# JasonLSC/GSCodec_Studio

Measured on AMD Instinct MI355X. Metric: Msplats/s fwd+bwd @1080p (1M splats), higher is better.
Workload: dtype f32; 1 GPU; BASELINE config 2: load_test_data(scene_grid=3) -> 1006065 gaussians, SH degree 3, 1x1 camera 1920x1080, packed=False, tile 16, fwd + bwd of sum(render); visible=292931, native_step_driver=True, parallelism=camera-sharded dp1

## Files before the change

gscodec_studio_amd/csrc/gs_common.h:

```cpp
#pragma once

#include <hip/hip_runtime.h>
#include <stdint.h>

#include "../../include/gsplat_hip.h"

#define GS_WAVE 64
#define GS_BLOCK 256

#define GS_DEV __device__ __forceinline__
#define GS_FP_STRICT _Pragma("clang fp contract(off)")

void gs_set_error(const char *fmt, ...);

#define GS_CHECK_ARG(cond, msg)                                                        \
    do {                                                                               \
        if (!(cond)) {                                                                 \
            gs_set_error("%s: %s", __func__, msg);                                     \
            return 1;                                                                  \
        }                                                                              \
    } while (0)

#define GS_CHECK_LAUNCH()                                                              \
    do {                                                                               \
        hipError_t e_ = hipGetLastError();                                             \
        if (e_ != hipSuccess) {                                                        \
            gs_set_error("%s: launch failed: %s", __func__, hipGetErrorString(e_));    \
            return 2;                                                                  \
        }                                                                              \
    } while (0)

static inline uint32_t gs_div_up(uint64_t a, uint64_t b) { return (uint32_t)((a + b - 1) / b); }

#define GS_PRESORT_BUCKETS 256
#ifdef __HIPCC__
__device__ __forceinline__ uint32_t gs_bucket_of(const uint64_t *s_split, uint64_t key) {
    uint32_t lo = 0;
#pragma unroll
    for (uint32_t step = GS_PRESORT_BUCKETS / 2; step >= 1; step >>= 1)
        if (s_split[lo + step - 1] <= key) lo += step;
    return lo;
}
#endif

#ifdef __HIPCC__
__device__ __forceinline__ float gs_mask_sigmoid(float v) { return __fdiv_rn(1.f, __fadd_rn(1.f, expf(-v))); }
__device__ __forceinline__ float gs_mask_value(float logit, float temperature, int binary) {
    if (binary) return gs_mask_sigmoid(logit) >= 0.5f ? 1.f : 0.f;
    return gs_mask_sigmoid(__fdiv_rn(logit, temperature));
}
#endif

#ifdef __HIPCC__
struct TileBox {
    int32_t x0, y0, x1, y1;
};
__device__ __forceinline__ TileBox tile_box(float mx, float my, int32_t radius, float tile_size, int32_t tw, int32_t th) {
    _Pragma("clang fp contract(off)");
    const float tr = ((float)radius / tile_size);
    const float tx = (mx / tile_size);
    const float ty = (my / tile_size);
    TileBox b;
    b.x0 = min(max(0, (int32_t)floorf((tx - tr))), tw);
    b.y0 = min(max(0, (int32_t)floorf((ty - tr))), th);
    b.x1 = min(max(0, (int32_t)ceilf((tx + tr))), tw);
    b.y1 = min(max(0, (int32_t)ceilf((ty + tr))), th);
    return b;
}
#endif

uint32_t *sort_first_hist_slot(uint64_t n, void *temp, size_t temp_bytes, uint32_t *n_blocks);

struct Vec3 {
    float x, y, z;
};
struct Mat3 {
    float m[3][3];
};
struct Sym3 {
    float xx, xy, xz, yy, yz, zz;
};
struct Sym2 {
    float xx, xy, yy;
};

GS_DEV Mat3 mat3_zero() {
    Mat3 r;
#pragma unroll
    for (int i = 0; i < 3; ++i)
#pragma unroll
        for (int j = 0; j < 3; ++j) r.m[i][j] = 0.f;
    return r;
}

GS_DEV Mat3 sym3_to_mat3(const Sym3 &s) {
    Mat3 r;
    r.m[0][0] = s.xx; r.m[0][1] = s.xy; r.m[0][2] = s.xz;
    r.m[1][0] = s.xy; r.m[1][1] = s.yy; r.m[1][2] = s.yz;
    r.m[2][0] = s.xz; r.m[2][1] = s.yz; r.m[2][2] = s.zz;
    return r;
}

GS_DEV Mat3 mat3_mul(const Mat3 &a, const Mat3 &b) {
    Mat3 r;
#pragma unroll
    for (int i = 0; i < 3; ++i)
#pragma unroll
        for (int j = 0; j < 3; ++j)
            r.m[i][j] = a.m[i][0] * b.m[0][j] + a.m[i][1] * b.m[1][j] + a.m[i][2] * b.m[2][j];
    return r;
}

GS_DEV Mat3 mat3_tmul(const Mat3 &a, const Mat3 &b) {
    Mat3 r;
#pragma unroll
    for (int i = 0; i < 3; ++i)
#pragma unroll
        for (int j = 0; j < 3; ++j)
            r.m[i][j] = a.m[0][i] * b.m[0][j] + a.m[1][i] * b.m[1][j] + a.m[2][i] * b.m[2][j];
    return r;
}

GS_DEV Mat3 mat3_mult(const Mat3 &a, const Mat3 &b) {
    Mat3 r;
#pragma unroll
    for (int i = 0; i < 3; ++i)
#pragma unroll
        for (int j = 0; j < 3; ++j)
            r.m[i][j] = a.m[i][0] * b.m[j][0] + a.m[i][1] * b.m[j][1] + a.m[i][2] * b.m[j][2];
    return r;
}

GS_DEV Sym3 sym3_congruence(const Mat3 &W, const Sym3 &S) {
    Mat3 Sm = sym3_to_mat3(S);
    Mat3 WS = mat3_mul(W, Sm);
    Sym3 r;
    r.xx = WS.m[0][0] * W.m[0][0] + WS.m[0][1] * W.m[0][1] + WS.m[0][2] * W.m[0][2];
    r.xy = WS.m[0][0] * W.m[1][0] + WS.m[0][1] * W.m[1][1] + WS.m[0][2] * W.m[1][2];
    r.xz = WS.m[0][0] * W.m[2][0] + WS.m[0][1] * W.m[2][1] + WS.m[0][2] * W.m[2][2];
    r.yy = WS.m[1][0] * W.m[1][0] + WS.m[1][1] * W.m[1][1] + WS.m[1][2] * W.m[1][2];
    r.yz = WS.m[1][0] * W.m[2][0] + WS.m[1][1] * W.m[2][1] + WS.m[1][2] * W.m[2][2];
    r.zz = WS.m[2][0] * W.m[2][0] + WS.m[2][1] * W.m[2][1] + WS.m[2][2] * W.m[2][2];
    return r;
}

GS_DEV Sym3 sym3_congruence_t(const Mat3 &W, const Sym3 &G) {
    Mat3 Gm = sym3_to_mat3(G);
    Mat3 GW = mat3_mul(Gm, W);
    Sym3 r;
    r.xx = W.m[0][0] * GW.m[0][0] + W.m[1][0] * GW.m[1][0] + W.m[2][0] * GW.m[2][0];
    r.xy = W.m[0][0] * GW.m[0][1] + W.m[1][0] * GW.m[1][1] + W.m[2][0] * GW.m[2][1];
    r.xz = W.m[0][0] * GW.m[0][2] + W.m[1][0] * GW.m[1][2] + W.m[2][0] * GW.m[2][2];
    r.yy = W.m[0][1] * GW.m[0][1] + W.m[1][1] * GW.m[1][1] + W.m[2][1] * GW.m[2][1];
    r.yz = W.m[0][1] * GW.m[0][2] + W.m[1][1] * GW.m[1][2] + W.m[2][1] * GW.m[2][2];
// ... 94 lines not shown
```

gscodec_studio_amd/csrc/isect.hip:

```cpp
#include "gs_common.h"

namespace {

__global__ void __launch_bounds__(GS_BLOCK) isect_count_kernel(
    uint32_t n_elems, const float *__restrict__ means2d, uint32_t s_m2, const int32_t *__restrict__ radii,
    float tile_size, int32_t tw, int32_t th, int32_t *__restrict__ tiles_per_gauss) {
    uint32_t i = blockIdx.x * GS_BLOCK + threadIdx.x;
    if (i >= n_elems) return;
    int32_t r = radii[i];
    int32_t cnt = 0;
    if (r > 0) {
        float2 m = *reinterpret_cast<const float2 *>(means2d + (size_t)i * s_m2);
        TileBox b = tile_box(m.x, m.y, r, tile_size, tw, th);
        cnt = (b.y1 - b.y0) * (b.x1 - b.x0);
    }
    tiles_per_gauss[i] = cnt;
}

__global__ void __launch_bounds__(GS_BLOCK) isect_depth_keys_kernel(
    uint32_t n_elems, const int32_t *__restrict__ radii, const float *__restrict__ depths,
    int64_t *__restrict__ keys, int32_t *__restrict__ vals) {
    uint32_t i = blockIdx.x * GS_BLOCK + threadIdx.x;
    if (i >= n_elems) return;
    uint32_t d = radii[i] > 0 ? (uint32_t)__float_as_int(depths[i]) & 0x7fffffffu : 0x7fffffffu;
    keys[i] = (int64_t)(((uint64_t)d << 32) | (uint64_t)i);
    vals[i] = (int32_t)i;
}

constexpr int COUNT_ITEMS = 4;
__global__ void __launch_bounds__(GS_BLOCK) isect_count_keys_kernel(
    uint32_t n_elems, const float *__restrict__ means2d, uint32_t s_m2, const int32_t *__restrict__ radii,
    const float *__restrict__ depths, float tile_size, int32_t tw, int32_t th,
    int32_t *__restrict__ tiles_per_gauss, int64_t *__restrict__ keys, int32_t *__restrict__ vals, int32_t *__restrict__ block_sums,
    uint32_t *__restrict__ hist, uint32_t n_blocks, const uint64_t *__restrict__ split) {
    __shared__ int32_t s_sum[GS_BLOCK / GS_WAVE], s_vis[GS_BLOCK / GS_WAVE];
    __shared__ uint32_t s_hist[256];
    __shared__ uint64_t s_split[GS_PRESORT_BUCKETS];
    if (hist != nullptr) s_hist[threadIdx.x] = 0u;
    if (split != nullptr) s_split[threadIdx.x] = split[threadIdx.x];
    __syncthreads();
    int32_t cnt_sum = 0, vis_sum = 0;
#pragma unroll
    for (int k = 0; k < COUNT_ITEMS; ++k) {
        const uint32_t i = (blockIdx.x * COUNT_ITEMS + k) * GS_BLOCK + threadIdx.x;
        if (i >= n_elems) continue;
        const int32_t r = radii[i];
        uint32_t d = 0x7fffffffu;
        int32_t cnt = 0;
        if (r > 0) {
            if (means2d != nullptr) {
                float2 m = *reinterpret_cast<const float2 *>(means2d + (size_t)i * s_m2);
                TileBox b = tile_box(m.x, m.y, r, tile_size, tw, th);
                cnt = (b.y1 - b.y0) * (b.x1 - b.x0);
            }
            d = (uint32_t)__float_as_int(depths[i]) & 0x7fffffffu;
        }
        if (means2d != nullptr) tiles_per_gauss[i] = cnt;
        const uint64_t key = ((uint64_t)d << 32) | (uint64_t)i;
        keys[i] = (int64_t)key;
        if (vals != nullptr) vals[i] = (int32_t)i;
        cnt_sum += cnt;
        vis_sum += r > 0 ? 1 : 0;
        if (hist != nullptr && d != 0x7fffffffu) atomicAdd(&s_hist[split != nullptr ? gs_bucket_of(s_split, key) : (d & 0xffu)], 1u);
    }
    if (block_sums != nullptr) {
        int32_t v = cnt_sum, u = vis_sum;
#pragma unroll
        for (int off = 32; off > 0; off >>= 1) {
            v += __shfl_xor(v, off, 64);
            u += __shfl_xor(u, off, 64);
        }
        if ((threadIdx.x & 63u) == 0u) {
            s_sum[threadIdx.x >> 6] = v;
            s_vis[threadIdx.x >> 6] = u;
        }
        __syncthreads();
        if (threadIdx.x == 0)
            reinterpret_cast<int2 *>(block_sums)[blockIdx.x] = make_int2(s_sum[0] + s_sum[1] + s_sum[2] + s_sum[3], s_vis[0] + s_vis[1] + s_vis[2] + s_vis[3]);
    }
    if (hist != nullptr) {
        __syncthreads();
        hist[(size_t)threadIdx.x * n_blocks + blockIdx.x] = s_hist[threadIdx.x];
    }
// ... 460 lines not shown
    hipLaunchKernelGGL(isect_emit_kernel<true>, dim3(gs_div_up(n_elems, EMIT_WAVES * EMIT_SPW)), dim3(GS_BLOCK), 0,
                       (hipStream_t)stream, n_elems, N, perm, n_valid, camera_ids, means2d, means2d_stride, radii, depths,
                       cum_tiles_per_gauss, (float)tile_size, (int32_t)tile_width, (int32_t)tile_height,
                       tile_n_bits, (int64_t *)nullptr, keys32, flatten_ids);
    GS_CHECK_LAUNCH();
    return 0;
}

extern "C" uint32_t gs_isect_emit_group_shift(void) { return EMIT_SCAN_SHIFT; }
extern "C" uint32_t gs_isect_emit_prefix_from_groups(void) { return 8192u; }

static int32_t emit_presorted_launch(
    int mode, uint32_t pos_bits, uint32_t n_elems, uint32_t N, const int32_t *perm, const uint32_t *n_valid, const int64_t *camera_ids,
    const float *means2d, uint32_t means2d_stride, const int32_t *radii, const float *depths, const int32_t *tiles_per_gauss,
    const uint32_t *group_sums, const int64_t *group_prefix, uint32_t tile_size, uint32_t tile_width, uint32_t tile_height,
    uint32_t tile_n_bits, int64_t *isect_ids, uint32_t *keys32, int32_t *flatten_ids, gs_stream_t stream) {
    const int32_t compact = mode != 0;
    if (n_elems == 0) return 0;
    GS_CHECK_ARG(means2d && radii && depths && tiles_per_gauss && (group_sums || group_prefix) && (flatten_ids || mode == 2), "null pointer");
    GS_CHECK_ARG(compact ? keys32 != nullptr : isect_ids != nullptr, "null output");
    GS_CHECK_ARG(camera_ids != nullptr || N > 0, "N must be > 0 when camera_ids is NULL");
    GS_CHECK_ARG(tile_n_bits < 32, "tile_n_bits must be < 32");
    GS_CHECK_ARG(means2d_stride >= 2 && means2d_stride % 2 == 0, "means2d_stride must be even and >= 2");
    GS_CHECK_ARG(n_elems < (1u << 31), "n_elems must be < 2^31");
    const dim3 grid(gs_div_up(n_elems, EMIT_SCAN_TILE));
    if (mode == 2)
        hipLaunchKernelGGL(isect_emit_scan_kernel<2>, grid, dim3(GS_BLOCK), 0, (hipStream_t)stream, n_elems, N, perm, n_valid, camera_ids,
                           means2d, means2d_stride, radii, depths, tiles_per_gauss, group_sums, group_prefix, (float)tile_size, (int32_t)tile_width,
                           (int32_t)tile_height, tile_n_bits, (int64_t *)nullptr, keys32, (int32_t *)nullptr, pos_bits);
    else if (compact)
        hipLaunchKernelGGL(isect_emit_scan_kernel<1>, grid, dim3(GS_BLOCK), 0, (hipStream_t)stream, n_elems, N, perm, n_valid, camera_ids,
                           means2d, means2d_stride, radii, depths, tiles_per_gauss, group_sums, group_prefix, (float)tile_size, (int32_t)tile_width,
                           (int32_t)tile_height, tile_n_bits, (int64_t *)nullptr, keys32, flatten_ids, 0u);
    else
        hipLaunchKernelGGL(isect_emit_scan_kernel<0>, grid, dim3(GS_BLOCK), 0, (hipStream_t)stream, n_elems, N, perm, n_valid, camera_ids,
                           means2d, means2d_stride, radii, depths, tiles_per_gauss, group_sums, group_prefix, (float)tile_size, (int32_t)tile_width,
                           (int32_t)tile_height, tile_n_bits, isect_ids, (uint32_t *)nullptr, flatten_ids, 0u);
    GS_CHECK_LAUNCH();
    return 0;
}

extern "C" int32_t gs_isect_emit_presorted(
    uint32_t n_elems, uint32_t N, const int32_t *perm, const uint32_t *n_valid, const int64_t *camera_ids, const float *means2d,
    uint32_t means2d_stride, const int32_t *radii, const float *depths, const int32_t *tiles_per_gauss, const uint32_t *group_sums,
    const int64_t *group_prefix, uint32_t tile_size, uint32_t tile_width, uint32_t tile_height, uint32_t tile_n_bits, int32_t compact,
    int64_t *isect_ids, uint32_t *keys32, int32_t *flatten_ids, gs_stream_t stream) {
    return emit_presorted_launch(compact ? 1 : 0, 0u, n_elems, N, perm, n_valid, camera_ids, means2d, means2d_stride, radii, depths,
                                 tiles_per_gauss, group_sums, group_prefix, tile_size, tile_width, tile_height, tile_n_bits, isect_ids, keys32,
                                 flatten_ids, stream);
}

extern "C" int32_t gs_isect_emit_packed(
    uint32_t n_elems, uint32_t N, const int32_t *perm, const uint32_t *n_valid, const int64_t *camera_ids, const float *means2d,
    uint32_t means2d_stride, const int32_t *radii, const float *depths, const int32_t *tiles_per_gauss, const uint32_t *group_sums,
    const int64_t *group_prefix, uint32_t tile_size, uint32_t tile_width, uint32_t tile_height, uint32_t tile_n_bits, uint32_t pos_bits,
    uint32_t *words, gs_stream_t stream) {
    GS_CHECK_ARG(pos_bits + tile_n_bits <= 32, "tile bits + position bits must fit 32 bits");
    return emit_presorted_launch(2, pos_bits, n_elems, N, perm, n_valid, camera_ids, means2d, means2d_stride, radii, depths, tiles_per_gauss,
                                 group_sums, group_prefix, tile_size, tile_width, tile_height, tile_n_bits, nullptr, words, nullptr, stream);
}

extern "C" int32_t gs_isect_offset_encode(
    uint32_t n_isects, const int64_t *isect_ids_sorted, uint32_t C, uint32_t n_tiles,
    uint32_t tile_n_bits, int32_t *offsets, gs_stream_t stream) {
    GS_CHECK_ARG(offsets != nullptr, "null pointer");
    if ((uint64_t)C * n_tiles == 0) return 0;
    if (n_isects == 0) {
        hipError_t e = hipMemsetAsync(offsets, 0, (size_t)C * n_tiles * sizeof(int32_t), (hipStream_t)stream);
        if (e != hipSuccess) {
            gs_set_error("gs_isect_offset_encode: memset failed: %s", hipGetErrorString(e));
            return 2;
        }
        return 0;
    }
    GS_CHECK_ARG(isect_ids_sorted != nullptr, "null pointer");
    hipLaunchKernelGGL(isect_offset_encode_kernel, dim3(gs_div_up(n_isects, GS_BLOCK * OFFSET_ITEMS)), dim3(GS_BLOCK), 0,
                       (hipStream_t)stream, n_isects, isect_ids_sorted, C, n_tiles, tile_n_bits, offsets);
    GS_CHECK_LAUNCH();
    return 0;
}

static size_t finish_pairs_bytes(uint64_t n) { return ((size_t)n * 4 + 255) / 256 * 256; }

extern "C" size_t gs_isect_finish_work_bytes(uint64_t n_isects) {
    return 2 * finish_pairs_bytes(n_isects) + gs_sort_isect_temp_bytes(n_isects);
}

extern "C" int32_t gs_isect_finish_presorted(
    uint32_t n_elems, uint32_t N, uint64_t n_isects, const int32_t *perm, const uint32_t *n_valid, const int64_t *camera_ids,
    const float *means2d, uint32_t means2d_stride, const int32_t *radii, const float *depths, const int32_t *tiles_per_gauss,
    const uint32_t *group_sums, const int64_t *group_prefix, uint32_t tile_size, uint32_t tile_width, uint32_t tile_height,
    uint32_t tile_n_bits, uint32_t cam_n_bits, uint32_t C, int64_t *isect_ids, int32_t *flatten_ids, int32_t *offsets, void *work,
    size_t work_bytes, uint32_t n_kept_host, const int64_t *sorted_keys, gs_stream_t stream) {
    GS_CHECK_ARG(offsets != nullptr, "null pointer");
    if (n_isects > 0) {
        GS_CHECK_ARG(work != nullptr && (uintptr_t)work % 16 == 0 && work_bytes >= gs_isect_finish_work_bytes(n_isects),
                     "work buffer too small (gs_isect_finish_work_bytes) or misaligned");
        const size_t pb = finish_pairs_bytes(n_isects);
        uint32_t *keys32 = (uint32_t *)work;
        int32_t *vals = (int32_t *)((char *)work + pb);
        void *temp = (char *)work + 2 * pb;
        uint32_t pos_bits = 0, cam_bits = 0;
        while (n_kept_host > 0 && ((uint64_t)1 << pos_bits) < (uint64_t)n_kept_host) ++pos_bits;
        while (((uint32_t)1 << cam_bits) < C) ++cam_bits;
        const uint32_t key_bits_eff = tile_n_bits + cam_bits;
        if (n_kept_host > 0 && perm != nullptr && camera_ids == nullptr && key_bits_eff >= 1 && key_bits_eff + pos_bits <= 32 &&
            key_bits_eff <= 31) {
            int32_t rc = gs_isect_emit_packed(n_elems, N, perm, n_valid, camera_ids, means2d, means2d_stride, radii, depths, tiles_per_gauss,
                                              group_sums, group_prefix, tile_size, tile_width, tile_height, tile_n_bits, pos_bits, keys32, stream);
            if (rc != 0) return rc;
            rc = gs_sort_isect_packed(n_isects, keys32, perm, sorted_keys, depths, (int32_t)key_bits_eff, pos_bits, isect_ids, flatten_ids,
                                      temp, work_bytes - 2 * pb, stream);
            if (rc != 0) return rc;
            return gs_isect_offset_encode((uint32_t)n_isects, isect_ids, C, tile_width * tile_height, tile_n_bits, offsets, stream);
        }
        int32_t rc = gs_isect_emit_presorted(n_elems, N, perm, n_valid, camera_ids, means2d, means2d_stride, radii, depths, tiles_per_gauss,
                                             group_sums, group_prefix, tile_size, tile_width, tile_height, tile_n_bits, 1, nullptr,
                                             keys32, vals, stream);
        if (rc != 0) return rc;
        const uint32_t sort_bits = (tile_n_bits + cam_n_bits < 32u && key_bits_eff >= 1u) ? key_bits_eff : tile_n_bits + cam_n_bits;
        rc = gs_sort_isect_pairs(n_isects, keys32, vals, depths, (int32_t)sort_bits, isect_ids, flatten_ids, temp,
                                 work_bytes - 2 * pb, stream);
        if (rc != 0) return rc;
    }
    return gs_isect_offset_encode((uint32_t)n_isects, isect_ids, C, tile_width * tile_height, tile_n_bits, offsets, stream);
}
```

gscodec_studio_amd/csrc/radix_sort.hip:

```cpp
#include "gs_common.h"

namespace {

constexpr int RADIX_BITS = 8;
constexpr int RADIX = 1 << RADIX_BITS;
constexpr int SORT_WAVES = GS_BLOCK / GS_WAVE;
constexpr int SORT_ROUNDS_BIG = 16, SORT_ROUNDS_SMALL = 4;
constexpr uint64_t SORT_SMALL_N = 2u << 20;
constexpr int sort_tile(int rounds) { return GS_BLOCK * rounds; }
inline int sort_rounds_for(uint64_t n) { return n <= SORT_SMALL_N ? SORT_ROUNDS_SMALL : SORT_ROUNDS_BIG; }

struct DigitSpec {
    uint32_t shift;
    uint32_t mask;
    uint32_t flip;
    uint32_t drop;
    uint32_t drop_hi;
    const uint64_t *split;
};

GS_DEV bool key_kept(uint64_t key, DigitSpec d) { return !(d.drop != 0u && (uint32_t)(key >> 32) == d.drop_hi); }
GS_DEV bool key_kept(uint32_t, DigitSpec) { return true; }

GS_DEV uint32_t digit_of(uint64_t key, DigitSpec d) { return ((uint32_t)(key >> d.shift) & d.mask) ^ d.flip; }
// ... 394 lines not shown
    GS_CHECK_ARG(begin_bit >= 0 && end_bit <= 64 && begin_bit <= end_bit, "bad bit range");
    GS_CHECK_ARG(n < (1ull << 32), "n must be < 2^32");
    int32_t rc = sort_impl(n, keys_in, vals_in, keys_out, vals_out, begin_bit, end_bit, false, 0u, nullptr, temp, temp_bytes,
                           (hipStream_t)stream, "gs_sort_pairs_u64_i32");
    if (rc) return rc;
    GS_CHECK_LAUNCH();
    return 0;
}

extern "C" int32_t gs_sort_pairs_u64_i32_drop(
    uint64_t n, const int64_t *keys_in, const int32_t *vals_in, int64_t *keys_out,
    int32_t *vals_out, int32_t begin_bit, int32_t end_bit, uint32_t drop_hi32, uint32_t *n_kept, void *temp,
    size_t temp_bytes, int32_t first_hist_ready, const int32_t *side_vals, uint32_t *side_sums, uint32_t side_shift,
    gs_stream_t stream) {
    if (n == 0) return 0;
    GS_CHECK_ARG(keys_in && vals_in && keys_out && vals_out && n_kept, "null pointer");
    GS_CHECK_ARG(begin_bit >= 0 && end_bit <= 64 && begin_bit < end_bit, "bad bit range");
    GS_CHECK_ARG(n < (1ull << 32), "n must be < 2^32");
    GS_CHECK_ARG(!first_hist_ready || (begin_bit == 32 && end_bit == 64), "a precomputed first histogram is defined for the bit range [32, 64)");
    GS_CHECK_ARG((side_vals == nullptr) == (side_sums == nullptr) && side_shift < 32, "side_vals and side_sums go together");
    int32_t rc = sort_impl(n, keys_in, vals_in, keys_out, vals_out, begin_bit, end_bit, true, drop_hi32, n_kept, temp, temp_bytes,
                           (hipStream_t)stream, "gs_sort_pairs_u64_i32_drop", first_hist_ready != 0, side_vals, side_sums, side_shift);
    if (rc) return rc;
    GS_CHECK_LAUNCH();
    return 0;
}

namespace {

struct Sort32Layout {
    uint32_t n_blocks;
    size_t off_keys, off_vals, off_hist, off_totals, total;
};

Sort32Layout sort32_layout(uint64_t n) {
    Sort32Layout L;
    L.n_blocks = gs_div_up(n, sort_tile(sort_rounds_for(n)));
    size_t o = 0;
    auto take = [&](size_t bytes) {
        size_t r = o;
        o += (bytes + 255) & ~(size_t)255;
        return r;
    };
    L.off_keys = take(n * sizeof(uint32_t));
    L.off_vals = take(n * sizeof(int32_t));
    L.off_hist = take((size_t)RADIX * L.n_blocks * sizeof(uint32_t));
    L.off_totals = take(RADIX * sizeof(uint32_t));
    L.total = o;
    return L;
}

template <int ROUNDS>
void launch_pass32(uint64_t n, const uint32_t *src_k, const int32_t *src_v, uint32_t *dst_k, int32_t *dst_v, DigitSpec d,
                   const Sort32Layout &L, uint32_t *hist, uint32_t *totals, bool final, const IsectEpilogue &ep, hipStream_t st) {
    hipLaunchKernelGGL((sort_hist_kernel<uint32_t, ROUNDS>), dim3(L.n_blocks), dim3(GS_BLOCK), 0, st, n, (const uint32_t *)nullptr, src_k, d, L.n_blocks, hist);
    hipLaunchKernelGGL(sort_scan_kernel, dim3(RADIX), dim3(GS_BLOCK), 0, st, L.n_blocks, hist, totals, (uint32_t *)nullptr, 0u);
    const ScatterSide none = {nullptr, nullptr, 0u};
    if (final)
        hipLaunchKernelGGL((sort_scatter_kernel<uint32_t, ROUNDS, true>), dim3(L.n_blocks), dim3(GS_BLOCK), 0, st, n, (const uint32_t *)nullptr, src_k, src_v,
                           dst_k, dst_v, d, L.n_blocks, hist, totals, (uint32_t *)nullptr, ep, none);
    else
        hipLaunchKernelGGL((sort_scatter_kernel<uint32_t, ROUNDS, false>), dim3(L.n_blocks), dim3(GS_BLOCK), 0, st, n, (const uint32_t *)nullptr, src_k, src_v,
                           dst_k, dst_v, d, L.n_blocks, hist, totals, (uint32_t *)nullptr, ep, none);
}

template <int ROUNDS>
void launch_pass32_keys(uint64_t n, const uint32_t *src_k, uint32_t *dst_k, DigitSpec d, const Sort32Layout &L, uint32_t *hist,
                        uint32_t *totals, bool final, const IsectEpilogue &ep, hipStream_t st) {
    hipLaunchKernelGGL((sort_hist_kernel<uint32_t, ROUNDS>), dim3(L.n_blocks), dim3(GS_BLOCK), 0, st, n, (const uint32_t *)nullptr, src_k, d, L.n_blocks, hist);
    hipLaunchKernelGGL(sort_scan_kernel, dim3(RADIX), dim3(GS_BLOCK), 0, st, L.n_blocks, hist, totals, (uint32_t *)nullptr, 0u);
    const ScatterSide none = {nullptr, nullptr, 0u};
    if (final)
        hipLaunchKernelGGL((sort_scatter_kernel<uint32_t, ROUNDS, true, false, true>), dim3(L.n_blocks), dim3(GS_BLOCK), 0, st, n, (const uint32_t *)nullptr,
                           src_k, (const int32_t *)nullptr, dst_k, (int32_t *)nullptr, d, L.n_blocks, hist, totals, (uint32_t *)nullptr, ep, none);
    else
        hipLaunchKernelGGL((sort_scatter_kernel<uint32_t, ROUNDS, false, false, true>), dim3(L.n_blocks), dim3(GS_BLOCK), 0, st, n, (const uint32_t *)nullptr,
                           src_k, (const int32_t *)nullptr, dst_k, (int32_t *)nullptr, d, L.n_blocks, hist, totals, (uint32_t *)nullptr, ep, none);
}

}

extern "C" size_t gs_sort_isect_temp_bytes(uint64_t n) { return sort32_layout(n).total; }

extern "C" int32_t gs_sort_isect_packed(uint64_t n, uint32_t *words, const int32_t *perm, const int64_t *sorted_keys, const float *depths,
                                        int32_t key_bits, uint32_t pos_bits, int64_t *isect_ids, int32_t *flatten_ids, void *temp,
                                        size_t temp_bytes, gs_stream_t stream) {
    if (n == 0) return 0;
    GS_CHECK_ARG(words && ((perm && depths) || sorted_keys) && isect_ids && flatten_ids, "null pointer");
    GS_CHECK_ARG(key_bits >= 1 && key_bits <= 31 && (uint32_t)key_bits + pos_bits <= 32, "key_bits (<= 31) + pos_bits must fit 32 bits");
    GS_CHECK_ARG(n < (1ull << 32), "n must be < 2^32");
    const Sort32Layout L = sort32_layout(n);
    if (temp == nullptr || temp_bytes < L.total) {
        gs_set_error("gs_sort_isect_packed: temp too small (%zu < %zu)", temp_bytes, L.total);
        return 1;
    }
    hipStream_t st = (hipStream_t)stream;
    char *tp = (char *)temp;
    uint32_t *tkeys = (uint32_t *)(tp + L.off_keys);
    uint32_t *hist = (uint32_t *)(tp + L.off_hist), *totals = (uint32_t *)(tp + L.off_totals);
    const int passes = (key_bits + RADIX_BITS - 1) / RADIX_BITS;
    const int first_bits = key_bits - (passes - 1) * RADIX_BITS;
    const IsectEpilogue ep = {depths, isect_ids, flatten_ids, perm, pos_bits, (const uint64_t *)sorted_keys};
    const bool small = sort_rounds_for(n) == SORT_ROUNDS_SMALL;
    const uint32_t *src_k = words;
    int shift = (int)pos_bits;
    for (int p = 0; p < passes; ++p) {
        DigitSpec d;
        const bool final = p == passes - 1;
        const int bits = (p == 0) ? first_bits : RADIX_BITS;
        d.shift = (uint32_t)shift;
        shift += bits;
        d.mask = (1u << bits) - 1u;
        d.drop = d.drop_hi = 0u;
        d.split = nullptr;
        d.flip = 0u;
        uint32_t *dst_k = (p % 2 == 0) ? tkeys : words;
        if (small) launch_pass32_keys<SORT_ROUNDS_SMALL>(n, src_k, dst_k, d, L, hist, totals, final, ep, st);
        else launch_pass32_keys<SORT_ROUNDS_BIG>(n, src_k, dst_k, d, L, hist, totals, final, ep, st);
        src_k = dst_k;
    }
    GS_CHECK_LAUNCH();
    return 0;
}

extern "C" int32_t gs_sort_isect_pairs(uint64_t n, uint32_t *keys32, int32_t *vals, const float *depths, int32_t key_bits,
                                       int64_t *isect_ids, int32_t *flatten_ids, void *temp, size_t temp_bytes, gs_stream_t stream) {
    if (n == 0) return 0;
    GS_CHECK_ARG(keys32 && vals && depths && isect_ids && flatten_ids, "null pointer");
    GS_CHECK_ARG(key_bits >= 1 && key_bits <= 32, "key_bits must be in [1, 32]");
    GS_CHECK_ARG(n < (1ull << 32), "n must be < 2^32");
    const Sort32Layout L = sort32_layout(n);
    if (temp == nullptr || temp_bytes < L.total) {
        gs_set_error("gs_sort_isect_pairs: temp too small (%zu < %zu)", temp_bytes, L.total);
        return 1;
    }
    hipStream_t st = (hipStream_t)stream;
    char *tp = (char *)temp;
    uint32_t *tkeys = (uint32_t *)(tp + L.off_keys);
    int32_t *tvals = (int32_t *)(tp + L.off_vals);
    uint32_t *hist = (uint32_t *)(tp + L.off_hist), *totals = (uint32_t *)(tp + L.off_totals);
    const int passes = (key_bits + RADIX_BITS - 1) / RADIX_BITS;
    const int first_bits = key_bits - (passes - 1) * RADIX_BITS;
    const IsectEpilogue ep = {depths, isect_ids, flatten_ids, nullptr, 0u, nullptr};
    const bool small = sort_rounds_for(n) == SORT_ROUNDS_SMALL;
    const uint32_t *src_k = keys32;
    const int32_t *src_v = vals;
    int shift = 0;
    for (int p = 0; p < passes; ++p) {
        DigitSpec d;
        const bool final = p == passes - 1;
        const int bits = (p == 0) ? first_bits : RADIX_BITS;
        d.shift = (uint32_t)shift;
        shift += bits;
        d.mask = (1u << bits) - 1u;
        d.drop = d.drop_hi = 0u;
        d.split = nullptr;
        d.flip = (key_bits == 32 && final) ? (1u << (bits - 1)) : 0u;
        uint32_t *dst_k = (p % 2 == 0) ? tkeys : keys32;
        int32_t *dst_v = (p % 2 == 0) ? tvals : vals;
        if (small) launch_pass32<SORT_ROUNDS_SMALL>(n, src_k, src_v, dst_k, dst_v, d, L, hist, totals, final, ep, st);
        else launch_pass32<SORT_ROUNDS_BIG>(n, src_k, src_v, dst_k, dst_v, d, L, hist, totals, final, ep, st);
        src_k = dst_k;
        src_v = dst_v;
    }
    GS_CHECK_LAUNCH();
    return 0;
// ... 517 lines not shown
```

include/gsplat_hip.h:

```cpp
#ifndef GSPLAT_HIP_H
#define GSPLAT_HIP_H

#include <stddef.h>
#include <stdint.h>

#ifdef __cplusplus
extern "C" {
#endif

#define GS_ABI_VERSION 6

#define GS_CAMERA_PINHOLE 0
#define GS_CAMERA_ORTHO 1
#define GS_CAMERA_FISHEYE 2

#define GS_QUANT_NOISE 0
#define GS_QUANT_ROUND 1
#define GS_ACT_NONE 0
#define GS_ACT_EXP 1
#define GS_ACT_SIGMOID 2

typedef void *gs_stream_t;

int32_t gs_version(void);
// ... 137 lines not shown
    float *v_coeffs, float *v_dirs, gs_stream_t stream);

int32_t gs_camera_centers(uint32_t C, const float *viewmats, float *campos, gs_stream_t stream);
int32_t gs_sh_view_fwd(
    uint32_t C, uint32_t N, uint32_t K, uint32_t degree,
    const float *means, const float *campos, int32_t campos_from_viewmats, const float *coeffs,
    const float *coeffs_rest ,
    const int32_t *radii,
    float *colors, uint32_t colors_stride ,
    const float *opacities , float *opacities_cn , gs_stream_t stream);
int32_t gs_sh_view_bwd(
    uint32_t C, uint32_t N, uint32_t K, uint32_t degree,
    const float *means, const float *campos, int32_t campos_from_viewmats, const float *coeffs, const float *coeffs_rest,
    const int32_t *radii,
    const float *colors_out, uint32_t colors_out_stride, const float *v_colors, uint32_t v_colors_stride,
    float *v_coeffs, float *v_coeffs_rest , float *v_means,
    const float *v_opacities_cn , uint32_t v_opacities_stride, float *v_opacities ,
    int32_t outputs_prefilled,
    gs_stream_t stream);

int32_t gs_isect_count(
    uint32_t n_elems,
    const float *means2d, uint32_t means2d_stride ,
    const int32_t *radii,
    uint32_t tile_size, uint32_t tile_width, uint32_t tile_height,
    int32_t *tiles_per_gauss,
    gs_stream_t stream);

size_t gs_cumsum_scratch_bytes(uint64_t n);
int32_t gs_cumsum_i32(
    uint64_t n, const int32_t *in, int64_t *out,
    void *scratch, size_t scratch_bytes, gs_stream_t stream);
int32_t gs_cumsum_i32_i32(
    uint64_t n, const int32_t *in, int32_t *out,
    void *scratch, size_t scratch_bytes, gs_stream_t stream);

int32_t gs_isect_depth_keys(
    uint32_t n_elems, const int32_t *radii, const float *depths,
    int64_t *keys, int32_t *vals, gs_stream_t stream);
int32_t gs_gather_i32(uint32_t n, const int32_t *src, const int32_t *idx, int32_t *out, gs_stream_t stream);
int32_t gs_isect_count_keys(
    uint32_t n_elems, const float *means2d , uint32_t means2d_stride, const int32_t *radii, const float *depths,
    uint32_t tile_size, uint32_t tile_width, uint32_t tile_height,
    int32_t *tiles_per_gauss, int64_t *keys, int32_t *vals ,
    int32_t *block_sums ,
    void *sort_temp, size_t sort_temp_bytes ,
    const int64_t *bucket_splitters ,
    gs_stream_t stream);
uint32_t gs_isect_count_blocks(uint32_t n_elems);
int32_t gs_cumsum_gather_i32(
    uint64_t n, const int32_t *in, const int32_t *idx, const uint32_t *n_valid ,
    int64_t *out, void *scratch, size_t scratch_bytes, gs_stream_t stream);

int32_t gs_isect_emit(
    uint32_t n_elems, uint32_t N,
    const int32_t *perm,
    const uint32_t *n_valid,
    const int64_t *camera_ids,
    const float *means2d, uint32_t means2d_stride, const int32_t *radii, const float *depths,
    const int64_t *cum_tiles_per_gauss,
    uint32_t tile_size, uint32_t tile_width, uint32_t tile_height,
    uint32_t tile_n_bits,
    int64_t *isect_ids,
    int32_t *flatten_ids,
    gs_stream_t stream);

int32_t gs_isect_emit_compact(
    uint32_t n_elems, uint32_t N, const int32_t *perm, const uint32_t *n_valid, const int64_t *camera_ids,
    const float *means2d, uint32_t means2d_stride, const int32_t *radii, const float *depths, const int64_t *cum_tiles_per_gauss,
    uint32_t tile_size, uint32_t tile_width, uint32_t tile_height, uint32_t tile_n_bits,
    uint32_t *keys32,
    int32_t *flatten_ids,
    gs_stream_t stream);
uint32_t gs_isect_emit_group_shift(void);
uint32_t gs_isect_emit_prefix_from_groups(void);
int32_t gs_isect_emit_presorted(
    uint32_t n_elems, uint32_t N, const int32_t *perm, const uint32_t *n_valid, const int64_t *camera_ids,
    const float *means2d, uint32_t means2d_stride, const int32_t *radii, const float *depths,
    const int32_t *tiles_per_gauss, const uint32_t *group_sums,
    const int64_t *group_prefix ,
    uint32_t tile_size, uint32_t tile_width, uint32_t tile_height, uint32_t tile_n_bits, int32_t compact,
    int64_t *isect_ids, uint32_t *keys32, int32_t *flatten_ids, gs_stream_t stream);
size_t gs_isect_finish_work_bytes(uint64_t n_isects);
int32_t gs_isect_finish_presorted(
    uint32_t n_elems, uint32_t N, uint64_t n_isects, const int32_t *perm, const uint32_t *n_valid, const int64_t *camera_ids,
    const float *means2d, uint32_t means2d_stride, const int32_t *radii, const float *depths,
    const int32_t *tiles_per_gauss, const uint32_t *group_sums, const int64_t *group_prefix,
    uint32_t tile_size, uint32_t tile_width, uint32_t tile_height, uint32_t tile_n_bits, uint32_t cam_n_bits, uint32_t C,
    int64_t *isect_ids , int32_t *flatten_ids , int32_t *offsets ,
    void *work, size_t work_bytes,
    uint32_t n_kept_host ,
    const int64_t *sorted_keys ,
    gs_stream_t stream);
int32_t gs_isect_emit_packed(
    uint32_t n_elems, uint32_t N, const int32_t *perm, const uint32_t *n_valid, const int64_t *camera_ids,
    const float *means2d, uint32_t means2d_stride, const int32_t *radii, const float *depths,
    const int32_t *tiles_per_gauss, const uint32_t *group_sums, const int64_t *group_prefix,
    uint32_t tile_size, uint32_t tile_width, uint32_t tile_height, uint32_t tile_n_bits, uint32_t pos_bits,
    uint32_t *words , gs_stream_t stream);
int32_t gs_sort_isect_packed(
    uint64_t n, uint32_t *words, const int32_t *perm, const int64_t *sorted_keys , const float *depths , int32_t key_bits,
    uint32_t pos_bits, int64_t *isect_ids, int32_t *flatten_ids, void *temp, size_t temp_bytes, gs_stream_t stream);
size_t gs_sort_isect_temp_bytes(uint64_t n);
int32_t gs_sort_isect_pairs(
    uint64_t n, uint32_t *keys32, int32_t *vals, const float *depths , int32_t key_bits,
    int64_t *isect_ids, int32_t *flatten_ids, void *temp, size_t temp_bytes, gs_stream_t stream);

size_t gs_sort_temp_bytes(uint64_t n);
int32_t gs_sort_pairs_u64_i32(
    uint64_t n,
    const int64_t *keys_in, const int32_t *vals_in,
    int64_t *keys_out, int32_t *vals_out,
    int32_t begin_bit, int32_t end_bit,
    void *temp, size_t temp_bytes, gs_stream_t stream);
int32_t gs_sort_pairs_u64_i32_drop(
    uint64_t n, const int64_t *keys_in, const int32_t *vals_in, int64_t *keys_out, int32_t *vals_out,
    int32_t begin_bit, int32_t end_bit, uint32_t drop_hi32, uint32_t *n_kept,
    void *temp, size_t temp_bytes,
    int32_t first_hist_ready ,
    const int32_t *side_vals, uint32_t *side_sums, uint32_t side_shift ,
    gs_stream_t stream);
int32_t gs_sort_first_hist_applicable(uint64_t n);

int32_t gs_presort_applicable(uint64_t n);
uint32_t gs_presort_capacity(void);
size_t gs_presort_temp_bytes(uint64_t n);
uint32_t gs_presort_split_elems(void);
int32_t gs_presort_split(
    uint32_t n_elems, const int32_t *radii, const float *depths, int64_t *splitters ,
    gs_stream_t stream);
int32_t gs_presort_buckets(
    uint64_t n, int64_t *keys_in , const int32_t *vals_in , const int64_t *splitters,
    int32_t *perm , uint32_t *n_kept ,
    void *temp, size_t temp_bytes, const int32_t *side_vals, uint32_t *side_sums, uint32_t side_shift,
    uint32_t lds_capacity, gs_stream_t stream);

int32_t gs_isect_offset_encode(
    uint32_t n_isects, const int64_t *isect_ids_sorted,
    uint32_t C, uint32_t n_tiles, uint32_t tile_n_bits,
    int32_t *offsets,
    gs_stream_t stream);

typedef struct gs_raster_plan {
    uint32_t magic, n_tiles_all, n_isects, channels;
    int32_t seg, solo_min;
    uint32_t xcd_fwd, xcd_bwd;
    uint64_t scratch_bytes;
    uint32_t reserved[6];
} gs_raster_plan;
int32_t gs_rasterize_plan(uint32_t n_tiles_all , uint32_t n_isects, uint32_t channels,
                          const int32_t *tuning , gs_raster_plan *plan);

int32_t gs_rasterize_fwd(
    uint32_t C, uint32_t n_elems, uint32_t n_isects, uint32_t channels,
    const float *means2d, const float *conics, const float *colors,
    const float *opacities,
    const uint32_t *splat_strides,
    const float *backgrounds,
    const uint8_t *masks,
    uint32_t image_width, uint32_t image_height, uint32_t tile_size,
    uint32_t tile_width, uint32_t tile_height,
    const int32_t *tile_offsets, const int32_t *flatten_ids,
    float *render_colors,
    float *render_alphas,
    int32_t *last_ids,
    const gs_raster_plan *plan, void *scratch,
// ... 334 lines not shown
```

Baseline: 1395 Msplats/s.

## Replace multi-pass radix sort of intersection keys with stable counting-sort tile binning

Adds a tile-binning path that handles the packed intersection keys with a per-chunk histogram, a cross-chunk scan and a scatter. The scatter does a two-pass 7-bit local LSD rank in shared memory to keep the scatter stable. Because the keys are already presorted by depth and the tile count (C * tiles, at most 16384) is small, one global counting pass replaces the multi-pass radix sort, and offsets are emitted directly without a separate encode kernel. The trade-offs are large per-chunk histogram rows (K+1 words per chunk) and heavy shared-memory use. The path is on by default with 16384-word chunks and can be switched off by an environment variable.

Measured after the change: 1412 Msplats/s, median of 6. 1.2% higher.

```diff
diff --git a/gscodec_studio_amd/csrc/gs_common.h b/gscodec_studio_amd/csrc/gs_common.h
--- a/gscodec_studio_amd/csrc/gs_common.h
+++ b/gscodec_studio_amd/csrc/gs_common.h
@@ -70,6 +70,14 @@
 #endif
 
 uint32_t *sort_first_hist_slot(uint64_t n, void *temp, size_t temp_bytes, uint32_t *n_blocks);
+size_t sort_isect_temp_bytes_bound(uint64_t n);
+
+constexpr uint32_t TB_CHUNK_MIN = 8192;
+constexpr uint32_t TB_KMAX = 16384;
+size_t tile_bin_temp_bytes(uint64_t n, uint32_t K);
+int32_t tile_bin_packed(uint64_t n, uint32_t chunk, const uint32_t *words, uint32_t pos_bits, uint32_t tile_n_bits, uint32_t n_tiles, uint32_t C,
+                        const int32_t *perm, const int64_t *sorted_keys, const float *depths, int64_t *isect_ids, int32_t *flatten_ids,
+                        int32_t *offsets, void *temp, size_t temp_bytes, hipStream_t st);
 
 struct Vec3 {
     float x, y, z;
diff --git a/gscodec_studio_amd/csrc/isect.hip b/gscodec_studio_amd/csrc/isect.hip
--- a/gscodec_studio_amd/csrc/isect.hip
+++ b/gscodec_studio_amd/csrc/isect.hip
@@ -1,4 +1,6 @@
 #include "gs_common.h"
+
+#include <stdlib.h>
 
 namespace {
 
@@ -625,8 +627,23 @@
 
 static size_t finish_pairs_bytes(uint64_t n) { return ((size_t)n * 4 + 255) / 256 * 256; }
 
+static int32_t tile_bin_default() {
+    const char *e = getenv("GS_TILE_BIN");
+    const int v = e != nullptr ? atoi(e) : -1;
+    return (v == 0 || v == 8192 || v == 16384) ? v : 16384;
+}
+static int32_t g_tile_bin_chunk = tile_bin_default();
+
+extern "C" int32_t gs_isect_tile_bin(int32_t chunk) {
+    const int32_t prev = g_tile_bin_chunk;
+    if (chunk == 0 || chunk == 8192 || chunk == 16384) g_tile_bin_chunk = chunk;
+    return prev;
+}
+
 extern "C" size_t gs_isect_finish_work_bytes(uint64_t n_isects) {
-    return 2 * finish_pairs_bytes(n_isects) + gs_sort_isect_temp_bytes(n_isects);
+    const size_t radix = 2 * finish_pairs_bytes(n_isects) + sort_isect_temp_bytes_bound(n_isects);
+    const size_t tiles = finish_pairs_bytes(n_isects) + tile_bin_temp_bytes(n_isects, TB_KMAX);
+    return radix > tiles ? radix : tiles;
 }
 
 extern "C" int32_t gs_isect_finish_presorted(
@@ -652,6 +669,10 @@
             int32_t rc = gs_isect_emit_packed(n_elems, N, perm, n_valid, camera_ids, means2d, means2d_stride, radii, depths, tiles_per_gauss,
                                               group_sums, group_prefix, tile_size, tile_width, tile_height, tile_n_bits, pos_bits, keys32, stream);
             if (rc != 0) return rc;
+            const uint64_t K = (uint64_t)C * tile_width * tile_height;
+            if (g_tile_bin_chunk != 0 && K >= 1 && K <= TB_KMAX && n_isects < (1ull << 31))
+                return tile_bin_packed(n_isects, (uint32_t)g_tile_bin_chunk, keys32, pos_bits, tile_n_bits, tile_width * tile_height, C, perm,
+                                       sorted_keys, depths, isect_ids, flatten_ids, offsets, (char *)work + pb, work_bytes - pb, (hipStream_t)stream);
             rc = gs_sort_isect_packed(n_isects, keys32, perm, sorted_keys, depths, (int32_t)key_bits_eff, pos_bits, isect_ids, flatten_ids,
                                       temp, work_bytes - 2 * pb, stream);
             if (rc != 0) return rc;
diff --git a/gscodec_studio_amd/csrc/radix_sort.hip b/gscodec_studio_amd/csrc/radix_sort.hip
--- a/gscodec_studio_amd/csrc/radix_sort.hip
+++ b/gscodec_studio_amd/csrc/radix_sort.hip
@@ -500,6 +500,12 @@
 
 extern "C" size_t gs_sort_isect_temp_bytes(uint64_t n) { return sort32_layout(n).total; }
 
+size_t sort_isect_temp_bytes_bound(uint64_t n) {
+    auto pad = [](size_t b) { return (b + 255) & ~(size_t)255; };
+    return pad(n * sizeof(uint32_t)) + pad(n * sizeof(int32_t)) +
+           pad((size_t)RADIX * gs_div_up(n, sort_tile(SORT_ROUNDS_SMALL)) * sizeof(uint32_t)) + pad(RADIX * sizeof(uint32_t));
+}
+
 extern "C" int32_t gs_sort_isect_packed(uint64_t n, uint32_t *words, const int32_t *perm, const int64_t *sorted_keys, const float *depths,
                                         int32_t key_bits, uint32_t pos_bits, int64_t *isect_ids, int32_t *flatten_ids, void *temp,
                                         size_t temp_bytes, gs_stream_t stream) {
diff --git a/gscodec_studio_amd/csrc/tile_bin.hip b/gscodec_studio_amd/csrc/tile_bin.hip
--- /dev/null
+++ b/gscodec_studio_amd/csrc/tile_bin.hip
@@ -0,0 +1,274 @@
+#include "gs_common.h"
+
+namespace {
+
+constexpr uint32_t TB_THREADS = 1024;
+constexpr uint32_t TB_WAVES = TB_THREADS / GS_WAVE;
+constexpr uint32_t TB_DIGIT_BITS = 7;
+constexpr uint32_t TB_RADIX = 1u << TB_DIGIT_BITS;
+static_assert(TB_KMAX == 1u << (2 * TB_DIGIT_BITS), "two LSD passes cover every key");
+
+GS_DEV uint32_t tb_key_index(uint32_t w, uint32_t pos_bits, uint32_t tile_n_bits, uint32_t n_tiles) {
+    const uint32_t key = w >> pos_bits;
+    return (key >> tile_n_bits) * n_tiles + (key & ((1u << tile_n_bits) - 1u));
+}
+
+template <uint32_t CHUNK>
+__global__ void __launch_bounds__(TB_THREADS) tile_bin_hist_kernel(
+    uint32_t n, const uint32_t *__restrict__ words, uint32_t pos_bits, uint32_t tile_n_bits, uint32_t n_tiles, uint32_t K,
+    uint32_t kp, uint32_t *__restrict__ E) {
+    __shared__ uint32_t s_h[TB_KMAX];
+    __shared__ uint32_t s_scan[TB_WAVES];
+    constexpr uint32_t TB_ITEMS = CHUNK / TB_THREADS;
+    static_assert(CHUNK % (4 * TB_THREADS) == 0, "a chunk is a whole number of 16-byte loads per thread");
+    const uint32_t tid = threadIdx.x, lane = tid % GS_WAVE, wave = tid / GS_WAVE;
+    const uint32_t base = blockIdx.x * CHUNK;
+    const uint32_t cnt = min(n - base, CHUNK);
+    for (uint32_t k = tid; k < K; k += TB_THREADS) s_h[k] = 0u;
+    __syncthreads();
+    if (cnt == CHUNK && (reinterpret_cast<uintptr_t>(words) & 15u) == 0u) {
+        const uint4 *w4 = reinterpret_cast<const uint4 *>(words + base);
+        uint4 v[TB_ITEMS / 4];
+#pragma unroll
+        for (uint32_t r = 0; r < TB_ITEMS / 4; ++r) v[r] = w4[r * TB_THREADS + tid];
+#pragma unroll
+        for (uint32_t r = 0; r < TB_ITEMS / 4; ++r) {
+            atomicAdd(&s_h[tb_key_index(v[r].x, pos_bits, tile_n_bits, n_tiles)], 1u);
+            atomicAdd(&s_h[tb_key_index(v[r].y, pos_bits, tile_n_bits, n_tiles)], 1u);
+            atomicAdd(&s_h[tb_key_index(v[r].z, pos_bits, tile_n_bits, n_tiles)], 1u);
+            atomicAdd(&s_h[tb_key_index(v[r].w, pos_bits, tile_n_bits, n_tiles)], 1u);
+        }
+    } else {
+        for (uint32_t j = tid; j < cnt; j += TB_THREADS) atomicAdd(&s_h[tb_key_index(words[base + j], pos_bits, tile_n_bits, n_tiles)], 1u);
+    }
+    __syncthreads();
+    const uint32_t per = (K + TB_THREADS - 1) / TB_THREADS;
+    const uint32_t k0 = tid * per;
+    uint32_t sum = 0;
+    for (uint32_t k = k0; k < min(k0 + per, K); ++k) sum += s_h[k];
+    uint32_t inc = sum;
+#pragma unroll
+    for (int off = 1; off < 64; off <<= 1) {
+        const uint32_t o = __shfl_up(inc, off, 64);
+        if (lane >= (uint32_t)off) inc += o;
+    }
+    if (lane == GS_WAVE - 1) s_scan[wave] = inc;
+    __syncthreads();
+    uint32_t run = inc - sum;
+    for (uint32_t w = 0; w < wave; ++w) run += s_scan[w];
+    for (uint32_t k = k0; k < min(k0 + per, K); ++k) {
+        const uint32_t c = s_h[k];
+        s_h[k] = run;
+        run += c;
+    }
+    __syncthreads();
+    uint32_t *row = E + (size_t)blockIdx.x * kp;
+    for (uint32_t k = tid; k < kp; k += TB_THREADS) row[k] = k < K ? s_h[k] : cnt;
+}
+
+__global__ void __launch_bounds__(TB_THREADS) tile_bin_scan_kernel(
+    uint32_t n_chunks, uint32_t K, uint32_t kp, const uint32_t *__restrict__ E, uint32_t *__restrict__ G, int32_t *__restrict__ offsets) {
+    __shared__ uint32_t s_e[TB_WAVES][GS_WAVE], s_c[TB_WAVES][GS_WAVE];
+    const uint32_t tid = threadIdx.x, lane = tid % GS_WAVE, wave = tid / GS_WAVE;
+    const uint32_t k = blockIdx.x * GS_WAVE + lane;
+    const uint32_t per = (n_chunks + TB_WAVES - 1) / TB_WAVES;
+    const uint32_t c0 = min(wave * per, n_chunks), c1 = min(c0 + per, n_chunks);
+    const bool on = k < K;
+    uint32_t se = 0, sc = 0;
+    if (on) {
+#pragma unroll 4
+        for (uint32_t c = c0; c < c1; ++c) {
+            const uint32_t e0 = E[(size_t)c * kp + k], e1 = E[(size_t)c * kp + k + 1];
+            se += e0;
+            sc += e1 - e0;
+        }
+    }
+    s_e[wave][lane] = se;
+    s_c[wave][lane] = sc;
+    __syncthreads();
+    if (!on) return;
+    uint32_t S = 0, pre = 0;
+#pragma unroll
+    for (uint32_t w = 0; w < TB_WAVES; ++w) {
+        S += s_e[w][lane];
+        if (w < wave) pre += s_c[w][lane];
+    }
+    if (wave == 0) offsets[k] = (int32_t)S;
+#pragma unroll 4
+    for (uint32_t c = c0; c < c1; ++c) {
+        const uint32_t e0 = E[(size_t)c * kp + k], e1 = E[(size_t)c * kp + k + 1];
+        G[(size_t)c * kp + k] = S + pre - e0;
+        pre += e1 - e0;
+    }
+}
+
+struct TbKey {
+    uint32_t pos_bits, tile_n_bits, n_tiles;
+    GS_DEV uint32_t operator()(uint32_t w) const { return tb_key_index(w, pos_bits, tile_n_bits, n_tiles); }
+};
+template <uint32_t TB_ITEMS>
+GS_DEV void tb_rank(const uint32_t (&w)[TB_ITEMS], uint32_t valid, const TbKey &key, uint32_t shift, uint32_t bits,
+                    uint32_t (*s_cnt)[TB_RADIX], uint32_t *s_dbase, uint32_t *s_scan, uint32_t *s_w) {
+    const uint32_t tid = threadIdx.x, lane = tid % GS_WAVE, wave = tid / GS_WAVE;
+    const unsigned long long lt_mask = (lane == 0) ? 0ull : (~0ull >> (64 - lane));
+    for (uint32_t i = tid; i < TB_WAVES * TB_RADIX; i += TB_THREADS) (&s_cnt[0][0])[i] = 0u;
+    __syncthreads();
+    const uint32_t mask = (1u << bits) - 1u;
+    uint32_t rank[TB_ITEMS];
+#pragma unroll
+    for (uint32_t r = 0; r < TB_ITEMS; ++r) {
+        const bool v = (valid >> r) & 1u;
+        const uint32_t dg = (key(w[r]) >> shift) & mask;
+        unsigned long long peers = __ballot(v);
+#pragma unroll
+        for (uint32_t b = 0; b < TB_DIGIT_BITS; ++b) {
+            if (b >= bits) break;
+            const bool bit = (dg >> b) & 1u;
+            const unsigned long long m = __ballot(bit);
+            peers &= bit ? m : ~m;
+        }
+        const uint32_t before = __popcll(peers & lt_mask);
+        const uint32_t leader = v ? (uint32_t)__builtin_ctzll(peers) : lane;
+        uint32_t b0 = 0;
+        if (v && before == 0) b0 = atomicAdd(&s_cnt[wave][dg], (uint32_t)__popcll(peers));
+        rank[r] = (b0 + before) | (leader << 16);
+    }
+#pragma unroll
+    for (uint32_t r = 0; r < TB_ITEMS; ++r) {
+        const uint32_t leader = rank[r] >> 16;
+        const uint32_t lead = __shfl(rank[r] & 0xffffu, (int)leader, 64);
+        rank[r] = (rank[r] & 0xffffu) + (leader != lane ? lead : 0u);
+    }
+    __syncthreads();
+    uint32_t run = 0;
+    if (tid < TB_RADIX) {
+#pragma unroll
+        for (uint32_t w = 0; w < TB_WAVES; ++w) {
+            const uint32_t c = s_cnt[w][tid];
+            s_cnt[w][tid] = run;
+            run += c;
+        }
+    }
+    uint32_t inc = run;
+#pragma unroll
+    for (int off = 1; off < 64; off <<= 1) {
+        const uint32_t o = __shfl_up(inc, off, 64);
+        if (lane >= (uint32_t)off) inc += o;
+    }
+    if (tid < TB_RADIX && lane == GS_WAVE - 1) s_scan[wave] = inc;
+    __syncthreads();
+    if (tid < TB_RADIX) s_dbase[tid] = inc - run + (wave > 0 ? s_scan[0] : 0u);
+    __syncthreads();
+#pragma unroll
+    for (uint32_t r = 0; r < TB_ITEMS; ++r) {
+        const uint32_t dg = (key(w[r]) >> shift) & mask;
+        if ((valid >> r) & 1u) s_w[s_dbase[dg] + s_cnt[wave][dg] + rank[r]] = w[r];
+    }
+}
+static_assert(TB_RADIX == 2 * GS_WAVE, "the digit scan above spans two waves");
+
+template <uint32_t CHUNK>
+__global__ void __launch_bounds__(TB_THREADS) tile_bin_scatter_kernel(
+    uint32_t n, const uint32_t *__restrict__ words, uint32_t pos_bits, uint32_t tile_n_bits, uint32_t n_tiles, uint32_t key_bits,
+    uint32_t kp, const uint32_t *__restrict__ G, const uint64_t *__restrict__ sorted_keys, const int32_t *__restrict__ perm,
+    const float *__restrict__ depths, int64_t *__restrict__ isect_ids, int32_t *__restrict__ flatten_ids) {
+    __shared__ uint32_t s_w[CHUNK];
+    __shared__ uint32_t s_cnt[TB_WAVES][TB_RADIX];
+    __shared__ uint32_t s_dbase[TB_RADIX];
+    __shared__ uint32_t s_scan[TB_WAVES];
+    constexpr uint32_t TB_ITEMS = CHUNK / TB_THREADS;
+    static_assert(CHUNK % (4 * TB_THREADS) == 0, "a chunk is a whole number of 16-byte loads per thread");
+    const uint32_t tid = threadIdx.x, lane = tid % GS_WAVE, wave = tid / GS_WAVE;
+    const uint32_t base = blockIdx.x * CHUNK;
+    const uint32_t cnt = min(n - base, CHUNK);
+    const uint32_t wave_first = wave * GS_WAVE * TB_ITEMS;
+    const TbKey key = {pos_bits, tile_n_bits, n_tiles};
+    uint32_t w[TB_ITEMS], valid = 0;
+#pragma unroll
+    for (uint32_t r = 0; r < TB_ITEMS; ++r) {
+        const uint32_t j = wave_first + r * GS_WAVE + lane;
+        w[r] = j < cnt ? words[base + j] : 0u;
+        valid |= j < cnt ? (1u << r) : 0u;
+    }
+    const uint32_t lo_bits = min(key_bits, TB_DIGIT_BITS), hi_bits = key_bits - lo_bits;
+    tb_rank(w, valid, key, 0u, lo_bits, s_cnt, s_dbase, s_scan, s_w);
+    __syncthreads();
+    if (hi_bits > 0) {
+#pragma unroll
+        for (uint32_t r = 0; r < TB_ITEMS; ++r) {
+            const uint32_t j = wave_first + r * GS_WAVE + lane;
+            w[r] = j < cnt ? s_w[j] : 0u;
+        }
+        tb_rank(w, valid, key, lo_bits, hi_bits, s_cnt, s_dbase, s_scan, s_w);
+        __syncthreads();
+    }
+    const uint32_t *grow = G + (size_t)blockIdx.x * kp;
+    const uint32_t pmask = (1u << pos_bits) - 1u;
+#pragma unroll 4
+    for (uint32_t r = 0; r < TB_ITEMS; ++r) {
+        const uint32_t j = r * TB_THREADS + tid;
+        if (j >= cnt) break;
+        const uint32_t wj = s_w[j];
+        const uint32_t at = wj & pmask;
+        const uint32_t pos = grow[min(key(wj), kp - 1u)] + j;
+        if (pos >= n) continue;
+        int32_t v;
+        int64_t db;
+        if (sorted_keys != nullptr) {
+            const uint64_t sk = sorted_keys[at];
+            v = (int32_t)(uint32_t)sk;
+            db = (int64_t)(sk >> 32);
+        } else {
+            v = perm[at];
+            db = (int64_t)__float_as_int(depths[v]);
+        }
+        isect_ids[pos] = (int64_t)((uint64_t)(wj >> pos_bits) << 32) | db;
+        flatten_ids[pos] = v;
+    }
+}
+
+static size_t tb_pad(size_t b) { return (b + 255) & ~(size_t)255; }
+static uint32_t tb_row(uint32_t K) { return (K + 1 + 63) / 64 * 64; }
+
+}
+
+size_t tile_bin_temp_bytes(uint64_t n, uint32_t K) {
+    const size_t chunks = n == 0 ? 0 : (size_t)gs_div_up(n, TB_CHUNK_MIN);
+    return 2 * tb_pad(chunks * tb_row(K) * sizeof(uint32_t));
+}
+
+template <uint32_t CHUNK>
+static void tile_bin_launch(uint64_t n, const uint32_t *words, uint32_t pos_bits, uint32_t tile_n_bits, uint32_t n_tiles, uint32_t K,
+                            const int32_t *perm, const int64_t *sorted_keys, const float *depths, int64_t *isect_ids, int32_t *flatten_ids,
+                            int32_t *offsets, void *temp, hipStream_t st) {
+    uint32_t key_bits = 0;
+    while ((1u << key_bits) < K) ++key_bits;
+    const uint32_t chunks = gs_div_up(n, CHUNK), kp = tb_row(K);
+    uint32_t *E = (uint32_t *)temp;
+    uint32_t *G = (uint32_t *)((char *)temp + tb_pad((size_t)chunks * kp * sizeof(uint32_t)));
+    hipLaunchKernelGGL(tile_bin_hist_kernel<CHUNK>, dim3(chunks), dim3(TB_THREADS), 0, st, (uint32_t)n, words, pos_bits, tile_n_bits, n_tiles,
+                       K, kp, E);
+    hipLaunchKernelGGL(tile_bin_scan_kernel, dim3(gs_div_up(K, GS_WAVE)), dim3(TB_THREADS), 0, st, chunks, K, kp, (const uint32_t *)E, G, offsets);
+    hipLaunchKernelGGL(tile_bin_scatter_kernel<CHUNK>, dim3(chunks), dim3(TB_THREADS), 0, st, (uint32_t)n, words, pos_bits, tile_n_bits, n_tiles,
+                       key_bits, kp, (const uint32_t *)G, (const uint64_t *)sorted_keys, perm, depths, isect_ids, flatten_ids);
+}
+
+int32_t tile_bin_packed(uint64_t n, uint32_t chunk, const uint32_t *words, uint32_t pos_bits, uint32_t tile_n_bits, uint32_t n_tiles,
+                        uint32_t C, const int32_t *perm, const int64_t *sorted_keys, const float *depths, int64_t *isect_ids,
+                        int32_t *flatten_ids, int32_t *offsets, void *temp, size_t temp_bytes, hipStream_t st) {
+    const uint64_t K = (uint64_t)C * n_tiles;
+    GS_CHECK_ARG(n > 0 && n < (1ull << 31) && K >= 1 && K <= TB_KMAX, "tile binning: n or C * n_tiles out of range");
+    GS_CHECK_ARG(temp != nullptr && temp_bytes >= tile_bin_temp_bytes(n, (uint32_t)K), "tile binning: temp too small");
+    GS_CHECK_ARG(words != nullptr && isect_ids != nullptr && flatten_ids != nullptr && offsets != nullptr &&
+                 (sorted_keys != nullptr || (perm != nullptr && depths != nullptr)), "null pointer");
+    if (chunk == 8192u)
+        tile_bin_launch<8192u>(n, words, pos_bits, tile_n_bits, n_tiles, (uint32_t)K, perm, sorted_keys, depths, isect_ids, flatten_ids, offsets,
+                               temp, st);
+    else if (chunk == 16384u)
+        tile_bin_launch<16384u>(n, words, pos_bits, tile_n_bits, n_tiles, (uint32_t)K, perm, sorted_keys, depths, isect_ids, flatten_ids, offsets,
+                                temp, st);
+    else
+        GS_CHECK_ARG(false, "tile binning: chunk must be 8192 or 16384 words");
+    GS_CHECK_LAUNCH();
+    return 0;
+}
diff --git a/include/gsplat_hip.h b/include/gsplat_hip.h
--- a/include/gsplat_hip.h
+++ b/include/gsplat_hip.h
@@ -243,6 +243,7 @@
     uint32_t tile_size, uint32_t tile_width, uint32_t tile_height, uint32_t tile_n_bits, int32_t compact,
     int64_t *isect_ids, uint32_t *keys32, int32_t *flatten_ids, gs_stream_t stream);
 size_t gs_isect_finish_work_bytes(uint64_t n_isects);
+int32_t gs_isect_tile_bin(int32_t chunk);
 int32_t gs_isect_finish_presorted(
     uint32_t n_elems, uint32_t N, uint64_t n_isects, const int32_t *perm, const uint32_t *n_valid, const int64_t *camera_ids,
     const float *means2d, uint32_t means2d_stride, const int32_t *radii, const float *depths,
```
